# dalab/matrix-manifolds

Hardware: NVIDIA B200
Metric: spd4_pair_dist_grad_evals_per_sec (higher is better)
Workload: dtype f32

## Files before the change

matrix-manifolds_b200/csrc/gm_manifolds.cuh:

```cuda
#pragma once
#include "gm_math.cuh"

namespace gm {


template <typename T, int N, bool FAST_CHOL>
struct InvChol {
  T a[N * N];
  T l[N * N];
  T fa, fb, fc, fdet;
  GM_HD void run(const T (&x)[N * N]) {
    if constexpr (FAST_CHOL) {
      static_assert(N == 2, "closed-form Cholesky exists for 2x2 only");
      const T eps = (T)1e-8;
      T x00 = clamp_min(x[0], eps);
      fa = Num<T>::sqrt(x00);
      fb = x[1] / fa;
      fc = Num<T>::sqrt(x[3] - fb * fb + eps);
      fdet = clamp_min(fa * fc, eps);
      a[0] = fc / fdet; a[1] = (T)0; a[2] = -fb / fdet; a[3] = fa / fdet;
      l[0] = fa; l[1] = (T)0; l[2] = fb; l[3] = fc;
    } else {
      chol_lower<T, N>(x, l);
      tri_inv_lower<T, N>(l, a);
// ... 40 lines not shown
struct ClosedEig;

template <typename T>
struct ClosedEig<T, 2> {
  GM_HD static T run(const T (&m)[4], T wmin, T wmax, bool want_grad, T (&g)[4]) {
    const T eps = (T)1e-8;
    T a = m[0], b = m[3], c = m[1];
    T det = a * b - c * c;
    T h = (T)0.5 * (a + b);
    T delta = clamp_min(h * h - det, eps);
    T r = Num<T>::sqrt(delta);
    T e1 = clampv(h - r, wmin, wmax), e2 = clampv(h + r, wmin, wmax);
    T l1 = Num<T>::log(e1), l2 = Num<T>::log(e2);
    T phi = l1 * l1 + l2 * l2;
    if (want_grad) {
      T g1 = (T)2 * l1 / e1, g2 = (T)2 * l2 / e2;
      T sh = (T)0.5 * (g1 + g2);
      T dr = (g2 - g1) / (r + r);
      g[0] = sh + dr * (h - b);
      g[3] = sh + dr * (h - a);
      g[1] = g[2] = dr * c;
    }
    return phi;
  }
};

template <typename T>
struct ClosedEig<T, 3> {
  GM_HD static T run(const T (&m)[9], T wmin, T wmax, bool want_grad, T (&g)[9]) {
    const T eps = (T)1e-8;
    const T two_pi_3 = (T)2.0943951023931954923084289221863;
    T q = (m[0] + m[4] + m[8]) / (T)3;
    T y00 = m[0] - q, y11 = m[4] - q, y22 = m[8] - q;
    T y01 = m[1], y02 = m[2], y12 = m[5];
    T y10 = m[3], y20 = m[6], y21 = m[7];
    T ss = y00 * y00 + y01 * y01 + y02 * y02 + y10 * y10 + y11 * y11 + y12 * y12 + y20 * y20 + y21 * y21 +
           y22 * y22;
    T p = clamp_min(Num<T>::sqrt(ss / (T)6), eps);
    T det = y00 * y11 * y22 + (T)2 * y01 * y02 * y12 - y11 * y02 * y02 - y00 * y12 * y12 - y22 * y01 * y01;
    T den = (T)2 * p * p * p + eps;
    T r = clampv(det / den, (T)-1 + eps, (T)1 - eps);
    T phi3 = Num<T>::acos(r) / (T)3;
    T c1 = Num<T>::cos(phi3), c2 = Num<T>::cos(phi3 + two_pi_3);
    T e1 = q + (T)2 * p * c1;
    T e2 = q + (T)2 * p * c2;
    T e3 = (T)3 * q - e1 - e2;
    T f1 = clampv(e1, wmin, wmax), f2 = clampv(e2, wmin, wmax), f3 = clampv(e3, wmin, wmax);
    T l1 = Num<T>::log(f1), l2 = Num<T>::log(f2), l3 = Num<T>::log(f3);
    T phi = l1 * l1 + l2 * l2 + l3 * l3;
    if (want_grad) {
      T g1 = (T)2 * l1 / f1, g2 = (T)2 * l2 / f2, g3 = (T)2 * l3 / f3;
      T e1b = g1 - g3, e2b = g2 - g3;
      T qb = (T)3 * g3 + e1b + e2b;
      T pb = (T)2 * (e1b * c1 + e2b * c2);
      T s1 = Num<T>::sin(phi3), s2 = Num<T>::sin(phi3 + two_pi_3);
      T phib = -(T)2 * p * (e1b * s1 + e2b * s2);
      T rb = -phib / ((T)3 * Num<T>::sqrt((T)1 - r * r));
      T detb = rb / den;
      pb += -rb * (det / den) / den * (T)6 * p * p;
      T ssb = pb / ((T)2 * p) / (T)6;
      T two_ssb = ssb + ssb;
      T b00 = two_ssb * y00 + detb * (y11 * y22 - y12 * y12);
      T b11 = two_ssb * y11 + detb * (y00 * y22 - y02 * y02);
      T b22 = two_ssb * y22 + detb * (y00 * y11 - y01 * y01);
      T b01 = two_ssb * y01 + detb * ((T)2 * y02 * y12 - (T)2 * y22 * y01);
      T b02 = two_ssb * y02 + detb * ((T)2 * y01 * y12 - (T)2 * y11 * y02);
      T b12 = two_ssb * y12 + detb * ((T)2 * y01 * y02 - (T)2 * y00 * y12);
      T b10 = two_ssb * y10, b20 = two_ssb * y20, b21 = two_ssb * y21;
      T dq = (qb - (b00 + b11 + b22)) / (T)3;
      g[0] = b00 + dq; g[4] = b11 + dq; g[8] = b22 + dq;
      g[1] = g[3] = (T)0.5 * (b01 + b10);
      g[2] = g[6] = (T)0.5 * (b02 + b20);
      g[5] = g[7] = (T)0.5 * (b12 + b21);
    }
    return phi;
  }
};

template <typename T, int N, bool FAST_EIG, bool FAST_CHOL>
struct SpdAI {
  static constexpr int E = N * N;
  T wmin, wmax;

  GM_HD T dist2(const T (&x)[E], const T (&y)[E]) const {
    InvChol<T, N, FAST_CHOL> ic;
    ic.run(x);
    T m[E];
    congr_lower<T, N>(ic.a, y, m);
    T phi;
    if constexpr (FAST_EIG) {
      T dummy[E];
      phi = ClosedEig<T, N>::run(m, wmin, wmax, false, dummy);
    } else {
      T v[E], w[N];
      jacobi_eigh<T, N, false>(m, v, w);
      phi = (T)0;
      if constexpr (FAST_CHOL) {
        GM_UNROLL for (int k = 0; k < N; ++k) {
          T lg = Num<T>::log(clampv(w[k], wmin, wmax));
          phi += lg * lg;
        }
      } else {
        const T lo = Num<T>::max(wmin, Num<T>::tiny), hi = Num<T>::min(wmax, Num<T>::huge);
        GM_UNROLL for (int k = 0; k < N; ++k) {
          T lg = Num<T>::log_pos(clampv(w[k], lo, hi));
          phi += lg * lg;
        }
      }
    }
    return clamp_min(phi, wmin);
  }

  static constexpr bool kCanPrep = !FAST_EIG && !FAST_CHOL;
  static constexpr int kPrepSize = N * (N + 1) / 2;
  struct EigState {
    T wm[E];
    T cx[N], cy[N];
  };
  GM_HD void prep(const T (&x)[E], T (&ap)[kPrepSize]) const {
    InvChol<T, N, false> ic;
    ic.run(x);
    GM_UNROLL for (int i = 0; i < N; ++i)
      GM_UNROLL for (int j = 0; j <= i; ++j) ap[i * (i + 1) / 2 + j] = ic.a[i * N + j];
  }
  GM_HD T eig_forward(const T (&a)[E], const T (&y)[E], EigState& st, int max_sweeps = JacobiCfg<T>::max_sweeps,
                      bool* converged = nullptr) const {
    T m[E], w[N];
    congr_lower<T, N>(a, y, m);
    GM_UNROLL for (int i = 0; i < N; ++i)
      GM_UNROLL for (int j = 0; j < N; ++j) st.wm[i * N + j] = (j >= i) ? a[j * N + i] : (T)0;
    const bool conv = jacobi_eigh<T, N, true, false>(m, st.wm, w, max_sweeps);
    if (converged) *converged = conv;
    T phi = (T)0;
    const T lo = Num<T>::max(wmin, Num<T>::tiny), hi = Num<T>::min(wmax, Num<T>::huge);
    GM_UNROLL for (int k = 0; k < N; ++k) {
      T wc = clampv(w[k], lo, hi);
      T lg = Num<T>::log_pos(wc);
      phi += lg * lg;
      T c = Num<T>::div_fast(lg + lg, wc);
      st.cy[k] = c;
      st.cx[k] = -c * w[k];
    }
    return clamp_min(phi, wmin);
  }
  GM_HD T eig_forward_prepped(const T (&ap)[kPrepSize], const T (&y)[E], EigState& st,
                              int max_sweeps = JacobiCfg<T>::max_sweeps, bool* converged = nullptr) const {
    T a[E];
    GM_UNROLL for (int i = 0; i < N; ++i)
      GM_UNROLL for (int j = 0; j < N; ++j) a[i * N + j] = (j <= i) ? ap[i * (i + 1) / 2 + j] : (T)0;
    return eig_forward(a, y, st, max_sweeps, converged);
  }
  GM_HD void eig_backward(const EigState& st, T wgt, T (&gx)[E], T (&gy)[E]) const {
    T cx[N], cy[N];
    GM_UNROLL for (int k = 0; k < N; ++k) { cx[k] = st.cx[k] * wgt; cy[k] = st.cy[k] * wgt; }
    wdwt<T, N>(st.wm, cx, gx);
    wdwt<T, N>(st.wm, cy, gy);
  }

  GM_HD T dist2_grad(const T (&x)[E], const T (&y)[E], T (&gx)[E], T (&gy)[E]) const {
    InvChol<T, N, FAST_CHOL> ic;
    ic.run(x);
    T m[E];
    congr_lower<T, N>(ic.a, y, m);
    T phi = (T)0;
    if constexpr (!FAST_EIG && !FAST_CHOL) {
      EigState st;
      T d2 = eig_forward(ic.a, y, st);
      eig_backward(st, (T)1, gx, gy);
      return d2;
    } else {
      T g[E];
      if constexpr (FAST_EIG) {
        phi = ClosedEig<T, N>::run(m, wmin, wmax, true, g);
      } else {
        T mm[E], v[E], w[N], c[N];
        GM_UNROLL for (int k = 0; k < E; ++k) mm[k] = m[k];
        jacobi_eigh<T, N, true>(mm, v, w);
        phi = (T)0;
        GM_UNROLL for (int k = 0; k < N; ++k) {
          T wc = clampv(w[k], wmin, wmax);
          T lg = Num<T>::log(wc);
          phi += lg * lg;
          c[k] = (T)2 * lg / wc;
        }
        wdwt<T, N>(v, c, g);
      }
      congr_lowerT<T, N>(ic.a, g, gy);
      if constexpr (FAST_CHOL) {
        T ga[E], abar[E];
        matmul<T, N>(g, ic.a, ga);
        matmul<T, N>(ga, y, abar);
        GM_UNROLL for (int k = 0; k < E; ++k) abar[k] *= (T)2;
        ic.backward_closed(abar, gx);
      } else {
        T k[E], pm[E];
        matmul<T, N>(g, m, k);
        GM_UNROLL for (int i = 0; i < N; ++i)
          GM_UNROLL for (int j = 0; j <= i; ++j) {
            pm[i * N + j] = -k[i * N + j];
            pm[j * N + i] = -k[i * N + j];
          }
        congr_lowerT<T, N>(ic.a, pm, gx);
      }
    }
    return clamp_min(phi, wmin);
  }
};

template <typename T, int N, bool FAST_CHOL>
struct SpdStein {
  static constexpr int E = N * N;
  static constexpr bool kCanPrep = false;
  static constexpr int kPrepSize = 1;
  T wmin, wmax;
  struct EigState {};
  GM_HD void prep(const T (&)[E], T (&)[1]) const {}
  GM_HD T eig_forward_prepped(const T (&)[1], const T (&)[E], EigState&, int = 0, bool* = nullptr) const { return (T)0; }
  GM_HD void eig_backward(const EigState&, T, T (&)[E], T (&)[E]) const {}

  template <bool WANT_INV>
  GM_HD static T logdet_inv(const T (&x)[E], T (&inv)[E]) {
    InvChol<T, N, FAST_CHOL> ic;
    ic.run(x);
    T ld = (T)0;
    GM_UNROLL for (int k = 0; k < N; ++k) ld += Num<T>::log(Num<T>::abs(ic.l[k * N + k]));
    if (WANT_INV) {
      GM_UNROLL for (int i = 0; i < N; ++i)
        GM_UNROLL for (int j = i; j < N; ++j) {
          T s = (T)0;
          GM_UNROLL for (int k = j; k < N; ++k) s += ic.a[k * N + i] * ic.a[k * N + j];
          inv[i * N + j] = s;
          inv[j * N + i] = s;
        }
    }
    return (T)2 * ld;
  }

  GM_HD T dist2(const T (&x)[E], const T (&y)[E]) const {
    T z[E], dummy[E];
// ... 138 lines not shown
      return d * d;
    } else if constexpr (KIND == VEC_SPHERE) {
      T s = (T)0;
      for (int k = 0; k < n; ++k) s += x[k] * y[k];
      s = clampv(s, -one_m, one_m);
      T d = clamp_min(Num<T>::acos(s), eps);
      c = -(T)2 * d / Num<T>::sqrt((T)1 - s * s);
      return d * d;
    } else if constexpr (KIND == VEC_EUCLIDEAN) {
      T s = (T)0;
      for (int k = 0; k < n; ++k) { T d = y[k] - x[k]; s += d * d; }
      c = (T)2;
      return clamp_min(s, eps);
    } else {
      const T cc = *c_dev;
      c = cc;
      T x2 = (T)0, y2 = (T)0, xy = (T)0;
      for (int k = 0; k < n; ++k) { x2 += x[k] * x[k]; y2 += y[k] * y[k]; xy += x[k] * y[k]; }
      const T A = (T)1 - (T)2 * cc * xy + cc * y2;
      const T B = (T)1 - cc * x2;
      const T D = (T)1 - (T)2 * cc * xy + cc * cc * x2 * y2;
      const bool d_free = D >= (T)Kappa<T>::kMinNorm;
      const T invD = (T)1 / clamp_min(D, (T)Kappa<T>::kMinNorm);
      co.zA = -A * invD;
      co.zB = B * invD;
      T r2 = (T)0, zx = (T)0, zy = (T)0;
      for (int k = 0; k < n; ++k) {
        T z = co.zA * x[k] + co.zB * y[k];
        r2 += z * z; zx += z * x[k]; zy += z * y[k];
      }
      const T r = Num<T>::sqrt(r2);
      const T sc = Num<T>::sqrt(Num<T>::abs(cc));
      T dphi;
      const T phi = Kappa<T>::arctan_func(sc * r, cc, dphi);
      const T d = phi * (T)2 / sc;
      const T d2 = d * d;
      const T gz = (r > (T)0) ? (T)4 * d * dphi / r : (T)0;
      const T dA = -(gz * zx) * invD;
      const T dB = (gz * zy) * invD;
      const T dD = d_free ? -(gz * r2) * invD : (T)0;
      const T g_xy = -(T)2 * cc * (dA + dD);
      const T g_x2 = -cc * dB + cc * cc * y2 * dD;
      const T g_y2 = cc * dA + cc * cc * x2 * dD;
      co.p1 = co.zA * gz; co.p2 = (T)2 * g_x2; co.p3 = g_xy;
      co.q1 = co.zB * gz; co.q2 = (T)2 * g_y2;
      const T sgn = cc > (T)0 ? (T)1 : (T)-1;
      const T w = cc * r2;
      T explicit_c;
      if (sizeof(T) == 4 && Num<T>::abs(w) < (T)0.1) {
        T sres = (T)0;
        GM_UNROLL for (int k = 8; k >= 1; --k) sres = sres * w + (T)(2.0 * k / (2.0 * k + 1.0));
        explicit_c = (T)2 * d * r * r2 * sres;
      } else {
        explicit_c = ((T)4 * d * dphi * r - (T)2 * d2) / sc * (sgn * (T)0.5 / sc);
      }
      co.dc = dA * (y2 - (T)2 * xy) - dB * x2 + dD * ((T)2 * cc * x2 * y2 - (T)2 * xy) + explicit_c;
      return clamp_min(d2, eps);
    }
  }
  GM_HD void grad_elem(int k, T xk, T yk, const VecCoef<T>& co, T& gxk, T& gyk) const {
    const T c = co.c;
    if constexpr (KIND == VEC_LORENTZ) {
      T sg = (k == 0) ? c : -c;
      gxk = sg * yk; gyk = sg * xk;
    } else if constexpr (KIND == VEC_SPHERE) {
      gxk = c * yk; gyk = c * xk;
    } else if constexpr (KIND == VEC_EUCLIDEAN) {
      T d = yk - xk;
      gxk = -c * d; gyk = c * d;
    } else {
      T z = co.zA * xk + co.zB * yk;
      gxk = co.p1 * z + co.p2 * xk + co.p3 * yk;
      gyk = co.q1 * z + co.q2 * yk + co.p3 * xk;
    }
  }
};

struct LossCfg {
  int kind, inc_l1, inc_l2;
  double alpha, eps;
};

template <typename T, bool FAST = false>
GM_HD T loss_term(const LossCfg& c, T g, T m, T& dm) {
  if (c.kind == 1) {
    T d = m - g;
    dm = (T)2 * d;
    return d * d;
  }
  T t = g * (T)c.alpha;
  T v = (T)0;
  dm = (T)0;
  if (c.inc_l1) {
    T rt = FAST ? Num<T>::div_fast((T)1, t) : (T)1 / t;
    T q = FAST ? m * rt - (T)1 : m / t - (T)1;
    v += Num<T>::abs(q);
    dm += sgn0(q) * rt;
  }
  if (c.inc_l2) {
    T den = m + (T)c.eps;
    T rd = FAST ? Num<T>::div_fast((T)1, den) : (T)1 / den;
    T q = FAST ? t * rd - (T)1 : t / den - (T)1;
    v += Num<T>::abs(q);
    dm -= FAST ? sgn0(q) * t * rd * rd : sgn0(q) * t / (den * den);
  }
  return v;
}

}
```

matrix-manifolds_b200/csrc/gm_math.cuh:

```cuda
#pragma once
#include <cuda_runtime.h>
#include <math.h>
#include <float.h>

#define GM_HD __host__ __device__ __forceinline__
#ifndef GM_ROT_NEWTON
#define GM_ROT_NEWTON 1
#endif

namespace gm {

template <typename T> struct Num;
template <> struct Num<float> {
  static constexpr float eps = FLT_EPSILON;
  static constexpr float tiny = FLT_MIN;
  static constexpr float huge = FLT_MAX;
  GM_HD static float sqrt(float x) { return sqrtf(x); }
  GM_HD static float rsqrt(float x) {
#ifdef __CUDA_ARCH__
    return rsqrtf(x);
#else
    return 1.0f / sqrtf(x);
#endif
  }
  GM_HD static float rsqrt_raw(float x) {
#ifdef __CUDA_ARCH__
    float r;
    asm("rsqrt.approx.ftz.f32 %0, %1;" : "=f"(r) : "f"(x));
    return r;
#else
    return 1.0f / sqrtf(x);
#endif
  }
  GM_HD static float rcp_raw(float x) {
#ifdef __CUDA_ARCH__
    float r;
    asm("rcp.approx.ftz.f32 %0, %1;" : "=f"(r) : "f"(x));
    return r;
#else
    return 1.0f / x;
#endif
  }
  GM_HD static float div_fast(float a, float b) { return a * rcp_raw(b); }
  GM_HD static float recip(float x) {
#ifdef __CUDA_ARCH__
    float r = rcp_raw(x);
    return fmaf(r, fmaf(-x, r, 1.0f), r);
#else
    return 1.0f / x;
#endif
  }
  GM_HD static float mul_sign(float v, float d) {
#ifdef __CUDA_ARCH__
    return __uint_as_float(__float_as_uint(v) ^ (__float_as_uint(d) & 0x80000000u));
#else
    return std::signbit(d) ? -v : v;
#endif
  }
  GM_HD static void rotation(float d, float apq, float& t, float& c, float& s) {
    float two = apq + apq;
    float h2 = fmaf(two, two, fmaf(d, d, FLT_MIN));
    float h = h2 * rsqrt_raw(h2);
    float den = fabsf(d) + h;
    t = mul_sign(two, d) * rcp_raw(den);
    float x = fmaf(t, t, 1.0f);
    float r = rsqrt_raw(x);
#if GM_ROT_NEWTON
    c = r * fmaf(-0.5f * x, r * r, 1.5f);
#else
    c = r;
#endif
    s = t * c;
  }
  GM_HD static float log(float x) { return logf(x); }
  GM_HD static float log_pos(float x) {
#ifdef __CUDA_ARCH__
    int ix = __float_as_int(x);
    int e = (ix - 0x3f2aaaab) & 0xff800000;
    float m = fmaf(x, 0.0f, __int_as_float(ix - e));
    float f = m - 1.0f;
    float g = -0.12734152376651764f;
    g = fmaf(g, f, 0.13756538927555084f);
    g = fmaf(g, f, -0.12219617515802383f);
    g = fmaf(g, f, 0.1405421793460846f);
    g = fmaf(g, f, -0.16678093373775482f);
    g = fmaf(g, f, 0.2000732272863388f);
    g = fmaf(g, f, -0.24999839067459106f);
    g = fmaf(g, f, 0.33333271741867065f);
    g = fmaf(g, f, -0.5f);
    float r = fmaf(f, f * g, f);
    return fmaf((float)e, 1.1920928955078125e-07f * 0.693147180559945309f, r);
#else
    return logf(x);
#endif
  }
  GM_HD static float log1p(float x) { return log1pf(x); }
  GM_HD static float exp(float x) { return expf(x); }
  GM_HD static float acos(float x) { return acosf(x); }
  GM_HD static float atan(float x) { return atanf(x); }
  GM_HD static float tan(float x) { return tanf(x); }
  GM_HD static float tanh(float x) { return tanhf(x); }
  GM_HD static float cos(float x) { return cosf(x); }
  GM_HD static float sin(float x) { return sinf(x); }
  GM_HD static float cosh(float x) { return coshf(x); }
  GM_HD static float sinh(float x) { return sinhf(x); }
  GM_HD static float abs(float x) { return fabsf(x); }
  GM_HD static float fma(float a, float b, float c) { return fmaf(a, b, c); }
  GM_HD static float max(float a, float b) { return fmaxf(a, b); }
  GM_HD static float min(float a, float b) { return fminf(a, b); }
  GM_HD static float copysign(float a, float b) { return copysignf(a, b); }
};
template <> struct Num<double> {
  static constexpr double eps = DBL_EPSILON;
  static constexpr double tiny = DBL_MIN;
  static constexpr double huge = DBL_MAX;
  GM_HD static double sqrt(double x) { return ::sqrt(x); }
  GM_HD static double rsqrt(double x) { return 1.0 / ::sqrt(x); }
  GM_HD static double div_fast(double a, double b) { return a / b; }
  GM_HD static double recip(double x) { return 1.0 / x; }
  GM_HD static void rotation(double d, double apq, double& t, double& c, double& s) {
    double two = apq + apq;
    double den = fabs(d) + ::sqrt(d * d + two * two);
    t = (den > 0.0) ? (d >= 0.0 ? two : -two) / den : 0.0;
    c = 1.0 / ::sqrt(t * t + 1.0);
    s = t * c;
  }
  GM_HD static double log(double x) { return ::log(x); }
  GM_HD static double log_pos(double x) { return ::log(x); }
  GM_HD static double log1p(double x) { return ::log1p(x); }
  GM_HD static double exp(double x) { return ::exp(x); }
  GM_HD static double acos(double x) { return ::acos(x); }
  GM_HD static double atan(double x) { return ::atan(x); }
  GM_HD static double tan(double x) { return ::tan(x); }
  GM_HD static double tanh(double x) { return ::tanh(x); }
  GM_HD static double cos(double x) { return ::cos(x); }
  GM_HD static double sin(double x) { return ::sin(x); }
  GM_HD static double cosh(double x) { return ::cosh(x); }
  GM_HD static double sinh(double x) { return ::sinh(x); }
  GM_HD static double abs(double x) { return fabs(x); }
  GM_HD static double fma(double a, double b, double c) { return ::fma(a, b, c); }
  GM_HD static double max(double a, double b) { return fmax(a, b); }
  GM_HD static double min(double a, double b) { return fmin(a, b); }
  GM_HD static double copysign(double a, double b) { return ::copysign(a, b); }
};

template <typename T>
GM_HD T clampv(T x, T lo, T hi) {
  return x < lo ? lo : (x > hi ? hi : x);
}
template <typename T>
GM_HD T clamp_min(T x, T lo) { return x < lo ? lo : x; }
template <typename T>
GM_HD T clamp_max(T x, T hi) { return x > hi ? hi : x; }
template <typename T>
GM_HD T sgn0(T x) { return (T)((x > (T)0) - (x < (T)0)); }

#define GM_UNROLL _Pragma("unroll")

template <typename T, int N>
GM_HD void chol_lower(const T (&x)[N * N], T (&l)[N * N]) {
  GM_UNROLL for (int j = 0; j < N; ++j) {
    T s = x[j * N + j];
    GM_UNROLL for (int k = 0; k < j; ++k) s -= l[j * N + k] * l[j * N + k];
    T d = Num<T>::sqrt(s);
    l[j * N + j] = d;
    T inv = (T)1 / d;
    GM_UNROLL for (int i = j + 1; i < N; ++i) {
      T t = x[i * N + j];
      GM_UNROLL for (int k = 0; k < j; ++k) t -= l[i * N + k] * l[j * N + k];
      l[i * N + j] = t * inv;
    }
    GM_UNROLL for (int i = 0; i < j; ++i) l[i * N + j] = (T)0;
  }
}

template <typename T, int N>
GM_HD void tri_inv_lower(const T (&l)[N * N], T (&a)[N * N]) {
  GM_UNROLL for (int j = 0; j < N; ++j) {
    GM_UNROLL for (int i = 0; i < j; ++i) a[i * N + j] = (T)0;
    a[j * N + j] = (T)1 / l[j * N + j];
    GM_UNROLL for (int i = j + 1; i < N; ++i) {
      T s = (T)0;
      GM_UNROLL for (int k = j; k < i; ++k) s += l[i * N + k] * a[k * N + j];
      a[i * N + j] = -s / l[i * N + i];
    }
  }
}

template <typename T, int N>
GM_HD void congr_lower(const T (&a)[N * N], const T (&y)[N * N], T (&m)[N * N]) {
  T t[N * N];
  GM_UNROLL for (int i = 0; i < N; ++i)
    GM_UNROLL for (int j = 0; j < N; ++j) {
      T s = (T)0;
      GM_UNROLL for (int k = 0; k <= i; ++k) s += a[i * N + k] * y[k * N + j];
      t[i * N + j] = s;
    }
  GM_UNROLL for (int i = 0; i < N; ++i)
    GM_UNROLL for (int j = i; j < N; ++j) {
      T s = (T)0;
      GM_UNROLL for (int k = 0; k <= j; ++k) s += t[i * N + k] * a[j * N + k];
      m[i * N + j] = s;
      m[j * N + i] = s;
    }
}

template <typename T, int N>
GM_HD void congr_full(const T (&a)[N * N], const T (&y)[N * N], T (&m)[N * N]) {
  T t[N * N];
  GM_UNROLL for (int i = 0; i < N; ++i)
    GM_UNROLL for (int j = 0; j < N; ++j) {
      T s = (T)0;
      GM_UNROLL for (int k = 0; k < N; ++k) s += a[i * N + k] * y[k * N + j];
      t[i * N + j] = s;
    }
  GM_UNROLL for (int i = 0; i < N; ++i)
    GM_UNROLL for (int j = i; j < N; ++j) {
      T s = (T)0;
      GM_UNROLL for (int k = 0; k < N; ++k) s += t[i * N + k] * a[j * N + k];
      m[i * N + j] = s;
      m[j * N + i] = s;
    }
}

template <typename T, int N>
GM_HD void lowerT_mul(const T (&a)[N * N], const T (&v)[N * N], T (&w)[N * N]) {
  GM_UNROLL for (int i = 0; i < N; ++i)
    GM_UNROLL for (int j = 0; j < N; ++j) {
      T s = (T)0;
      GM_UNROLL for (int k = i; k < N; ++k) s += a[k * N + i] * v[k * N + j];
      w[i * N + j] = s;
    }
}

template <typename T, int N>
GM_HD void lower_mul(const T (&l)[N * N], const T (&v)[N * N], T (&w)[N * N]) {
  GM_UNROLL for (int i = 0; i < N; ++i)
    GM_UNROLL for (int j = 0; j < N; ++j) {
      T s = (T)0;
      GM_UNROLL for (int k = 0; k <= i; ++k) s += l[i * N + k] * v[k * N + j];
      w[i * N + j] = s;
    }
}

template <typename T, int N>
GM_HD void wdwt(const T (&w)[N * N], const T (&c)[N], T (&g)[N * N]) {
  GM_UNROLL for (int i = 0; i < N; ++i)
    GM_UNROLL for (int j = i; j < N; ++j) {
      T s = (T)0;
      GM_UNROLL for (int k = 0; k < N; ++k) s += (w[i * N + k] * c[k]) * w[j * N + k];
      g[i * N + j] = s;
      g[j * N + i] = s;
    }
}

template <typename T, int N>
GM_HD void matmul(const T (&a)[N * N], const T (&b)[N * N], T (&c)[N * N]) {
  GM_UNROLL for (int i = 0; i < N; ++i)
    GM_UNROLL for (int j = 0; j < N; ++j) {
      T s = (T)0;
      GM_UNROLL for (int k = 0; k < N; ++k) s += a[i * N + k] * b[k * N + j];
      c[i * N + j] = s;
    }
}

template <typename T> struct JacobiCfg;
#ifndef GM_JACOBI_F32_OFF
#define GM_JACOBI_F32_OFF 16.0f
#endif
#ifndef GM_JACOBI_F32_OFF_MAX_N
#define GM_JACOBI_F32_OFF_MAX_N 4
#endif
template <> struct JacobiCfg<float> {
  static constexpr int max_sweeps = 10;
  static constexpr float off_factor = GM_JACOBI_F32_OFF;
};
template <> struct JacobiCfg<double> {
  static constexpr int max_sweeps = 16;
  static constexpr double off_factor = 0.0625;
};

template <int N>
struct JacobiFirstCheck { static constexpr int value = N >= 4 ? 3 : (N == 3 ? 2 : 1); };

template <typename T, int N, bool WANT_V = true, bool INIT_V = true>
GM_HD bool jacobi_eigh(T (&a)[N * N], T (&v)[N * N], T (&w)[N], int max_sweeps = JacobiCfg<T>::max_sweeps) {
  if (WANT_V && INIT_V) {
    GM_UNROLL for (int i = 0; i < N; ++i)
      GM_UNROLL for (int j = 0; j < N; ++j) v[i * N + j] = (i == j) ? (T)1 : (T)0;
  }
  if (N == 1) { w[0] = a[0]; return true; }
  auto rotate = [&](const int p, const int q) {
    T apq = a[p * N + q];
    T t, c, s;
    Num<T>::rotation(a[q * N + q] - a[p * N + p], apq, t, c, s);
    if constexpr (N >= 5) {
      const T app = a[p * N + p], aqq = a[q * N + q], cs2 = (T)2 * c * s * apq;
      a[p * N + p] = c * c * app - cs2 + s * s * aqq;
      a[q * N + q] = s * s * app + cs2 + c * c * aqq;
    } else {
      a[p * N + p] = Num<T>::fma(-t, apq, a[p * N + p]);
      a[q * N + q] = Num<T>::fma(t, apq, a[q * N + q]);
    }
    a[p * N + q] = (T)0;
    a[q * N + p] = (T)0;
    GM_UNROLL for (int r = 0; r < N; ++r) {
      if (r != p && r != q) {
        T arp = a[r * N + p], arq = a[r * N + q];
        T nrp = c * arp - s * arq;
        T nrq = s * arp + c * arq;
        a[r * N + p] = nrp; a[p * N + r] = nrp;
        a[r * N + q] = nrq; a[q * N + r] = nrq;
      }
    }
    if (WANT_V) {
      GM_UNROLL for (int r = 0; r < N; ++r) {
        T vrp = v[r * N + p], vrq = v[r * N + q];
        v[r * N + p] = c * vrp - s * vrq;
        v[r * N + q] = s * vrp + c * vrq;
      }
    }
  };
  bool converged = false;
  for (int sweep = 0;; ++sweep) {
    if (sweep >= JacobiFirstCheck<N>::value || sweep >= max_sweeps) {
      T off = (T)0, dia = (T)0;
      GM_UNROLL for (int i = 0; i < N; ++i) {
        dia += a[i * N + i] * a[i * N + i];
        GM_UNROLL for (int j = i + 1; j < N; ++j) off += a[i * N + j] * a[i * N + j];
      }
      constexpr T off_factor = (N <= GM_JACOBI_F32_OFF_MAX_N) ? JacobiCfg<T>::off_factor : (T)0.0625;
      converged = off <= (Num<T>::eps * Num<T>::eps * off_factor) * dia || off < Num<T>::tiny;
      if (converged || sweep >= max_sweeps) break;
    }
    if constexpr (N == 4) {
      rotate(0, 1); rotate(2, 3);
      rotate(0, 2); rotate(1, 3);
      rotate(0, 3); rotate(1, 2);
    } else {
      GM_UNROLL for (int p = 0; p < N - 1; ++p)
        GM_UNROLL for (int q = p + 1; q < N; ++q) rotate(p, q);
    }
  }
  GM_UNROLL for (int i = 0; i < N; ++i) w[i] = a[i * N + i];
  return converged;
}

template <typename T, int R, int C>
GM_HD void jacobi_svd(T (&a)[R * C], T (&v)[C * C], T (&s)[C]) {
  GM_UNROLL for (int i = 0; i < C; ++i)
    GM_UNROLL for (int j = 0; j < C; ++j) v[i * C + j] = (i == j) ? (T)1 : (T)0;
  for (int sweep = 0; sweep < JacobiCfg<T>::max_sweeps + 4; ++sweep) {
    bool rotated = false;
    GM_UNROLL for (int p = 0; p < C - 1; ++p) {
      GM_UNROLL for (int q = p + 1; q < C; ++q) {
        T alpha = (T)0, beta = (T)0, gamma = (T)0;
        GM_UNROLL for (int r = 0; r < R; ++r) {
          alpha += a[r * C + p] * a[r * C + p];
          beta += a[r * C + q] * a[r * C + q];
          gamma += a[r * C + p] * a[r * C + q];
        }
        if (Num<T>::abs(gamma) > (Num<T>::eps * (T)0.25) * Num<T>::sqrt(alpha * beta) &&
            Num<T>::abs(gamma) > Num<T>::tiny) {
          rotated = true;
          T t, c, sn;
          Num<T>::rotation(beta - alpha, gamma, t, c, sn);
          GM_UNROLL for (int r = 0; r < R; ++r) {
            T x = a[r * C + p], y = a[r * C + q];
            a[r * C + p] = c * x - sn * y;
            a[r * C + q] = sn * x + c * y;
          }
          GM_UNROLL for (int r = 0; r < C; ++r) {
            T x = v[r * C + p], y = v[r * C + q];
            v[r * C + p] = c * x - sn * y;
            v[r * C + q] = sn * x + c * y;
          }
        }
      }
    }
    if (!rotated) break;
  }
  GM_UNROLL for (int k = 0; k < C; ++k) {
    T n2 = (T)0;
    GM_UNROLL for (int r = 0; r < R; ++r) n2 += a[r * C + k] * a[r * C + k];
    s[k] = Num<T>::sqrt(n2);
  }
}

template <typename T>
__device__ __forceinline__ T warp_sum(T v) {
  GM_UNROLL for (int o = 16; o > 0; o >>= 1) v += __shfl_xor_sync(0xffffffffu, v, o);
  return v;
}

__device__ __forceinline__ void block_accumulate(double v, double* dst, double* red) {
  v = warp_sum(v);
  int lane = threadIdx.x & 31, wid = threadIdx.x >> 5;
  if (lane == 0) red[wid] = v;
  __syncthreads();
  if (wid == 0) {
    int nw = (blockDim.x + 31) >> 5;
    double s = lane < nw ? red[lane] : 0.0;
    s = warp_sum(s);
    if (lane == 0 && dst != nullptr) atomicAdd(dst, s);
  }
  __syncthreads();
}

}
```

matrix-manifolds_b200/csrc/gm_pairs_spd.cu:

```cuda
#include "gm_product.cuh"

#ifndef GM_N
#error "compile with -DGM_N=<matrix size>"
#endif

namespace gm {

template <class Op, typename T, int KMODE>
__global__ void __launch_bounds__(128)
spd_pair_kernel(Op op, PairSpec ps, const T* __restrict__ xa, const T* __restrict__ xb,
                const T* __restrict__ gout, T coef, T* __restrict__ ga, T* __restrict__ gb,
                T* __restrict__ out_d2, TargetSpec tg, LossCfg lc, T scale_sp, double* __restrict__ acc) {
  constexpr int E = Op::E;
  __shared__ double red[2][4];
  long long k = (long long)blockIdx.x * blockDim.x + threadIdx.x;
  bool active = k < ps.P;
  long long ra = -1, rb = -1;
  double loss_v = 0.0, gd2_v = 0.0;
  T gx[E], gy[E];
  if (active) {
    decode_pair(ps, k, ra, rb);
    T x[E], y[E];
    load_row<T, E>(xa, ra, x);
    load_row<T, E>(xb, rb, y);
    if constexpr (KMODE == K_FWD) {
      out_d2[k] = op.dist2(x, y);
    } else {
      T d2 = op.dist2_grad(x, y, gx, gy);
      T w;
      if constexpr (KMODE == K_BWD) {
        w = coef * gout[k];
      } else {
        T g = fetch_target_ps<T>(ps, tg, k, ra, rb);
        T m = scale_sp * d2;
        T dm;
        T lv = loss_term<T>(lc, g, m, dm);
        loss_v = (double)lv;
        gd2_v = (double)dm * (double)d2;
        w = dm * scale_sp;
        if (out_d2) out_d2[k] = d2;
      }
      GM_UNROLL for (int e = 0; e < E; ++e) { gx[e] *= w; gy[e] *= w; }
    }
  }
  if constexpr (KMODE != K_FWD) {
    if (ps.mode == GM_PAIRS_ELEMENTWISE) {
      if (active) {
        store_row<T, E>(ga, ra, gx);
        store_row<T, E>(gb, rb, gy);
      }
    } else {
      warp_accumulate_row<T, E>(ga, ra, gx);
      warp_accumulate_row<T, E>(gb, rb, gy);
    }
  }
  if constexpr (KMODE == K_FUSED) {
    block_accumulate(loss_v, acc, red[0]);
    block_accumulate(gd2_v, acc + 1, red[1]);
  }
}

template <int BYTES>
__device__ __forceinline__ void cp_async(void* smem, const void* gmem) {
  unsigned s = (unsigned)__cvta_generic_to_shared(smem);
  if constexpr (BYTES == 16)
    asm volatile("cp.async.cg.shared.global [%0], [%1], 16;\n" ::"r"(s), "l"(gmem) : "memory");
  else if constexpr (BYTES == 8)
    asm volatile("cp.async.ca.shared.global [%0], [%1], 8;\n" ::"r"(s), "l"(gmem) : "memory");
  else
    asm volatile("cp.async.ca.shared.global [%0], [%1], 4;\n" ::"r"(s), "l"(gmem) : "memory");
}
__device__ __forceinline__ void cp_async_commit() { asm volatile("cp.async.commit_group;\n" ::: "memory"); }
__device__ __forceinline__ void cp_async_wait_all() { asm volatile("cp.async.wait_group 0;\n" ::: "memory"); }
template <int PENDING>
__device__ __forceinline__ void cp_async_wait_group() { asm volatile("cp.async.wait_group %0;\n" ::"n"(PENDING) : "memory"); }

template <typename T, int E, int STAGES = 2>
struct RowStage {
  static constexpr int ROWB = E * (int)sizeof(T);
  static constexpr int CPB = (ROWB % 16 == 0) ? 16 : ((ROWB % 8 == 0) ? 8 : 4);
  static constexpr int NCH = ROWB / CPB;
  static constexpr int THREADS = 128;
  static constexpr int BYTES = STAGES * 2  * ROWB * THREADS;
  __device__ __forceinline__ static char* slot(char* base, int s, int r, int c, int t) {
    return base + ((((s * 2 + r) * NCH + c) * THREADS + t) * CPB);
  }
  __device__ __forceinline__ static void issue(char* base, int s, int r, int t, const T* row) {
    const char* g = reinterpret_cast<const char*>(row);
    GM_UNROLL for (int c = 0; c < NCH; ++c) cp_async<CPB>(slot(base, s, r, c, t), g + c * CPB);
  }
  __device__ __forceinline__ static void read(char* base, int s, int r, int t, T (&out)[E]) {
    GM_UNROLL for (int c = 0; c < NCH; ++c) {
      if constexpr (CPB == 16) {
        float4 v = *reinterpret_cast<const float4*>(slot(base, s, r, c, t));
        const T* tv = reinterpret_cast<const T*>(&v);
        GM_UNROLL for (int j = 0; j < 16 / (int)sizeof(T); ++j) out[c * (16 / (int)sizeof(T)) + j] = tv[j];
      } else if constexpr (CPB == 8) {
        float2 v = *reinterpret_cast<const float2*>(slot(base, s, r, c, t));
        const T* tv = reinterpret_cast<const T*>(&v);
        GM_UNROLL for (int j = 0; j < 8 / (int)sizeof(T); ++j) out[c * (8 / (int)sizeof(T)) + j] = tv[j];
      } else {
        out[c] = *reinterpret_cast<const T*>(slot(base, s, r, c, t));
      }
    }
  }
};

struct PairCursor {
  long long a, pos;
  int slot;
  __device__ __forceinline__ void init(const PairSpec& ps, long long k0) {
    if (ps.mode == GM_PAIRS_TRIU && k0 < ps.P) {
      long long b;
      triu_decode(k0 + ps.k0, ps.B, a, b);
      pos = b - a - 1;
    } else {
      a = -1; pos = 0; slot = 0;
    }
  }
// ... 171 lines not shown
    v[D] = locate(32 * D, kq);
    if (v[D]) load_rows(kq, ra[D], rb[D], hopn);
  }
  [[maybe_unused]] int hs = SPEC ? (32 * (D + 1)) / (int)chunk : 0;
  [[maybe_unused]] int ho = SPEC ? 32 * (D + 1) - hs * (int)chunk : 0;

  double loss_v = 0.0, gd2_v = 0.0;
  row_t acc_row = kNoRow;
  T gacc[EU];
  GM_UNROLL for (int e = 0; e < EU; ++e) gacc[e] = (T)0;
  row_t prep_row = kNoRow;
  T ap[Op::kPrepSize];

  auto flush = [&]() {
    if (acc_row != kNoRow) {
      GM_UNROLL for (int e = 0; e < EU; ++e) gacc[e] = warp_sum(gacc[e]);
      if (lane == 0) {
        T gfull[E];
        GM_UNROLL for (int i = 0; i < N; ++i)
          GM_UNROLL for (int j = i; j < N; ++j) {
            gfull[i * N + j] = gacc[i * N - i * (i - 1) / 2 + (j - i)];
            gfull[j * N + i] = gfull[i * N + j];
          }
        long long lr;
        T* gbase = grow(ga, acc_row, lr);
        atomic_add_row<T, E>(gbase, lr, gfull);
      }
      GM_UNROLL for (int e = 0; e < EU; ++e) gacc[e] = (T)0;
      acc_row = kNoRow;
    }
  };

  const int t_end = (nseg > 1 && wbase - lane < ps.seg_len) ? nseg * (int)chunk : 0;
  while (nseg > 1 ? tc < t_end : __any_sync(full, v[0])) {
    cp_async_wait_group<D - 1>();
    const bool v0 = v[0];
    const row_t ra0 = ra[0], rb0 = rb[0];
    const raw_t tg0 = tgq[0];
    T x[E], y[E];
    if (v0) {
      Stage::read(stage_mem, stage, 1, tid, y);
      if (!Op::kCanPrep || ra0 != prep_row) Stage::read(stage_mem, stage, 0, tid, x);
    }
    tgq[D] = 0;
    if (v[D]) {
      long long kq = 0;
      if (KMODE == K_BWD || !hopsP) locate(tc + 32 * D, kq);
      tgq[D] = (sampled && hopsP) ? (raw_t)hopn : fetch_scalar(kq, ra[D], rb[D]);
      if (rawj) rb[D] &= (row_t)0x00ffffffu;
      int sn = stage + D;
      if (sn > D) sn -= D + 1;
      Stage::issue(stage_mem, sn, 0, tid, xrow(xa, ra[D]));
      Stage::issue(stage_mem, sn, 1, tid, xrow(xb, rb[D]));
    }
    cp_async_commit();
    ahead.advance(ps);
    long long kh = 0;
    if constexpr (SPEC != 0) {
      v[D + 1] = locate_so(hs, ho, kh);
      ho += 32;
      if (ho >= (int)chunk) { ho -= (int)chunk; ++hs; }
    } else {
      v[D + 1] = locate(tc + 32 * (D + 1), kh);
    }
    ra[D + 1] = kNoRow; rb[D + 1] = kNoRow;
    unsigned hop_next = 0;
    if (v[D + 1]) load_rows(kh, ra[D + 1], rb[D + 1], hop_next);

    T gx[E], gy[E];
    if (v0) {
      T d2, w;
      [[maybe_unused]] typename Op::EigState st;
      if constexpr (Op::kCanPrep) {
        if (ra0 != prep_row) { op.prep(x, ap); prep_row = ra0; }
        d2 = op.eig_forward_prepped(ap, y, st);
      } else {
        d2 = op.dist2_grad(x, y, gx, gy);
      }
      if constexpr (KMODE == K_BWD) {
        w = coef * scalar_value(tg0);
      } else {
        T m = scale_sp * d2;
        T dm;
        T lv = loss_term<T, true>(lc, scalar_value(tg0), m, dm);
        loss_v += (double)lv;
        gd2_v += (double)dm * (double)d2;
        w = dm * scale_sp;
        if (out_d2) {
          long long k0 = 0;
          locate(tc, k0);
          out_d2[k0] = d2;
        }
      }
      if constexpr (Op::kCanPrep) {
        op.eig_backward(st, w, gx, gy);
      } else {
        GM_UNROLL for (int e = 0; e < E; ++e) { gx[e] *= w; gy[e] *= w; }
      }
      long long lrb;
      T* gbb = grow(gb, rb0, lrb);
      atomic_add_row<T, E>(gbb, lrb, gy);
    }
    {
      row_t r0 = __shfl_sync(full, ra0, 0);
      bool uniform = __all_sync(full, v0 && ra0 == r0);
      if (uniform && r0 == acc_row) {
        GM_UNROLL for (int i = 0; i < N; ++i)
          GM_UNROLL for (int j = i; j < N; ++j) gacc[i * N - i * (i - 1) / 2 + (j - i)] += gx[i * N + j];
      } else {
        flush();
        if (uniform) {
          acc_row = r0;
          GM_UNROLL for (int i = 0; i < N; ++i)
            GM_UNROLL for (int j = i; j < N; ++j) gacc[i * N - i * (i - 1) / 2 + (j - i)] = gx[i * N + j];
        } else if (v0) {
          long long lra;
          T* gba = grow(ga, ra0, lra);
          atomic_add_row<T, E>(gba, lra, gx);
        }
      }
    }
    tc += 32;
    GM_UNROLL for (int q = 0; q < D + 1; ++q) { ra[q] = ra[q + 1]; rb[q] = rb[q + 1]; v[q] = v[q + 1]; }
    GM_UNROLL for (int q = 0; q < D; ++q) tgq[q] = tgq[q + 1];
    hopn = hop_next;
    stage = (stage == D) ? 0 : stage + 1;
  }
  flush();
  if constexpr (KMODE == K_FUSED) {
    block_accumulate(loss_v, acc, red[0]);
    block_accumulate(gd2_v, acc + 1, red[1]);
  }
}

template <class Op, typename T>
static int launch_op(const Op& op, const PairArgs& a) {
  if (a.ps.P <= 0) return 0;
  if (a.px) return a.sh.log2w >= 0 ? GM_EUNSUPPORTED : launch_product<SpdLead<Op>, T>(SpdLead<Op>{op}, a);
  const int threads = 128;
  long long blocks = (a.ps.P + threads - 1) / threads;
  if (blocks > 0x7fffffffLL) return GM_EINVAL;
  dim3 grid((unsigned)blocks), block(threads);
  const T* xa = (const T*)a.xa;
  const T* xb = (const T*)a.xb;
#ifndef GM_MINB_F32
#define GM_MINB_F32 4
#endif
#ifndef GM_PF_DEPTH
#define GM_PF_DEPTH 1
#endif
  constexpr int MINB = sizeof(T) == 4 ? GM_MINB_F32 : 2;
  constexpr int DEPTH = (RowStage<T, Op::E, GM_PF_DEPTH + 1>::BYTES + 3 * 1024) * MINB <= 224 * 1024 ? GM_PF_DEPTH : 1;
  using Stage = RowStage<T, Op::E, DEPTH + 1>;
  if (a.kmode != K_FWD && a.ps.mode != GM_PAIRS_ELEMENTWISE && RowStage<T, Op::E, 2>::BYTES <= 64 * 1024) {
    int dev = 0, sms = 0, occ = 0;
    cudaGetDevice(&dev);
    cudaDeviceGetAttribute(&sms, cudaDevAttrMultiProcessorCount, dev);
    auto launch_stream = [&](auto kern, auto spec_kern, const T* gout, T coef, T* out_d2, T scale, double* acc) -> int {
      cudaFuncSetAttribute(kern, cudaFuncAttributeMaxDynamicSharedMemorySize, Stage::BYTES);
      cudaOccupancyMaxActiveBlocksPerMultiprocessor(&occ, kern, threads, Stage::BYTES);
      if (occ < 1) occ = 1;
      long long max_blocks = (long long)sms * occ;
      long long want = (a.ps.P + threads - 1) / threads;
      long long nb = want < max_blocks ? want : max_blocks;
      long long warps = nb * (threads / 32);
      PairSpec ps = a.ps;
      if (ps.mode != GM_PAIRS_LIST || ps.nseg < 2 || ps.P < ps.nseg * 32LL * warps) ps.nseg = 1;
// ... 83 lines not shown
```

Before: 15.25 billion.

## Use packed f32x2 FMA for 4x4 SPD congruence, eigvec rotations and backward

Adds an f32x2 type backed by Blackwell packed fma/mul/add.rn.f32x2 PTX. The 4x4 float SPD path uses it for a specialized congruence, Jacobi eigenvector rotations stored as row pairs, a two-lane polynomial log, and the W diag W^T gradient reconstruction, so two scalar FP32 operations issue as one instruction. It also changes the loss sign test to compensate for rounding error in m, and adds a diagnostic script. The risks are packing overhead through 64-bit moves, higher register pressure, and slightly different rounding from the custom log.

```diff
diff --git a/_diag.py b/_diag.py
--- /dev/null
+++ b/_diag.py
@@ -0,0 +1,45 @@
+import os, sys, torch
+sys.path[:0] = ['tests', 'oracle', 'matrix-manifolds_b200']
+import helpers_hotpath as H
+from graphembed import _ops, _lib as L
+from graphembed.manifolds import SymmetricPositiveDefinite
+DEV = torch.device('cuda', 0); MAX_SQ = 64.0
+S = float(torch.nn.functional.softplus(torch.tensor(0.5)))
+x, cls, _ = H.point_table(4, {H.CA: 2048, H.CB: 2048}, seed=21)
+gen = torch.Generator().manual_seed(22)
+B = 1536
+nodes = torch.randperm(x.shape[0], generator=gen)[:B]
+ia, ib = torch.triu_indices(B, B, 1)
+k0 = int(torch.nonzero(ia == 100)[0]) + 37
+P = ia.numel() - k0 - 1234
+I, J = nodes[ia[k0:k0 + P]], nodes[ib[k0:k0 + P]]
+h = torch.randint(1, 9, (x.shape[0], x.shape[0]), generator=gen, dtype=torch.uint8)
+h = torch.triu(h, 1) + torch.triu(h, 1).T
+ref = H.PairReference(x, I, J, 4)
+pcls = H.pair_classes(cls, I, J); rcls = H.row_classes(cls, (I, J), pcls)
+dense = (h.float() ** 2) / MAX_SQ
+xd = x.to(DEV)
+pairs = _ops.PairSet.triu(B, nodes=nodes.to(torch.int32).to(DEV), device=DEV, k0=k0, P=P)
+grad = torch.zeros_like(xd)
+acc, d2 = _ops.pairs_loss_fused(SymmetricPositiveDefinite(4).spec, xd, pairs, _ops.TargetSpec.dense(dense.to(DEV)),
+                                _ops.LossSpec(L.GM_LOSS_QUOTIENT, True, True, 1.0, 0.5), S, grad, want_d2=True)
+d2 = d2.cpu(); grad = grad.cpu()
+g = dense[I, J].double()
+w = H.loss_weights('quotient', g, d2, S)[2]
+chk = H.Checker(torch.float32, os.environ['TAG'])
+chk.grad([(grad, [(I, 'gx'), (J, 'gy')])], ref, w, [rcls])
+print(chk.report())
+g64 = torch.zeros(x.shape, dtype=torch.float64); A = torch.zeros(x.shape[0], dtype=torch.float64)
+for rows, side in ((I, 'gx'), (J, 'gy')):
+    c = w.view(-1, 1, 1) * getattr(ref, side + '_64'); g64.index_add_(0, rows, c); A.index_add_(0, rows, H._item_max(c))
+loc = H._item_max(grad.double() - g64) / A.clamp(min=1e-300)
+top = torch.topk(loc, 4)
+m64 = S * d2.double()
+q1 = m64 / g - 1.0; q2 = g / (m64 + 0.5) - 1.0
+near = (q1.abs() < 3e-6) | (q2.abs() < 3e-6)
+print('pairs within 3e-6 of a kink:', int(near.sum()))
+for r, v in zip(top.indices.tolist(), top.values.tolist()):
+    sel = near & ((I == r) | (J == r))
+    ks = torch.nonzero(sel).flatten().tolist()
+    info = [(k, f'q1={q1[k]:.2e}', f'q2={q2[k]:.2e}', f'|w contrib|/A={(w[k].abs() * H._item_max(ref.gx_64[k:k+1] if I[k]==r else ref.gy_64[k:k+1])[0] / A[r]).item():.2e}') for k in ks]
+    print(f'row {r} cls {int(rcls[r])} loc err {v:.2e} near-kink pairs {info}')
diff --git a/matrix-manifolds_b200/csrc/gm_manifolds.cuh b/matrix-manifolds_b200/csrc/gm_manifolds.cuh
--- a/matrix-manifolds_b200/csrc/gm_manifolds.cuh
+++ b/matrix-manifolds_b200/csrc/gm_manifolds.cuh
@@ -146,10 +146,20 @@
   static constexpr int E = N * N;
   T wmin, wmax;
 
+  static constexpr bool kPacked = sizeof(T) == 4 && N == 4 && !FAST_EIG && !FAST_CHOL;
+
   GM_HD T dist2(const T (&x)[E], const T (&y)[E]) const {
     InvChol<T, N, FAST_CHOL> ic;
     ic.run(x);
     T m[E];
+    if constexpr (kPacked) {
+      T ap[kPrepSize], v[E], w[N];
+      pack_factor(ic.a, ap);
+      congr4(ap, y, m);
+      jacobi_eigh<T, N, false>(m, v, w);
+      f32x2 wc[2], lg[2];
+      return clamp_min(log_pairs(w, wc, lg), wmin);
+    }
     congr_lower<T, N>(ic.a, y, m);
     T phi;
     if constexpr (FAST_EIG) {
@@ -177,18 +187,90 @@
 
   static constexpr bool kCanPrep = !FAST_EIG && !FAST_CHOL;
   static constexpr int kPrepSize = N * (N + 1) / 2;
-  struct EigState {
+  struct EigStateScalar {
     T wm[E];
     T cx[N], cy[N];
   };
+  struct EigStatePacked {
+    f32x2 wp[8];
+    f32x2 cx[2], cy[2];
+  };
+  using EigState = typename std::conditional<kPacked, EigStatePacked, EigStateScalar>::type;
+
+  GM_HD static void pack_factor(const T (&a)[E], T (&ap)[kPrepSize]) {
+    if constexpr (kPacked) {
+      const int src[kPrepSize] = {0, 4, 8, 12, 9, 13, 10, 14, 5, 15};
+      GM_UNROLL for (int e = 0; e < kPrepSize; ++e) ap[e] = a[src[e]];
+    } else {
+      GM_UNROLL for (int i = 0; i < N; ++i)
+        GM_UNROLL for (int j = 0; j <= i; ++j) ap[i * (i + 1) / 2 + j] = a[i * N + j];
+    }
+  }
+  GM_HD static void congr4(const float (&ap)[10], const float (&y)[16], float (&m)[16]) {
+    const f32x2 a0{ap[0], ap[1]}, b0{ap[2], ap[3]}, b1{ap[4], ap[5]}, b2{ap[6], ap[7]};
+    const float a11 = ap[8], a33 = ap[9];
+    f32x2 t0[4], t1[4];
+    GM_UNROLL for (int j = 0; j < 4; ++j) {
+      t0[j] = mul2(a0, y[j]);
+      t0[j].y = fmaf(a11, y[4 + j], t0[j].y);
+      t1[j] = fma2(b2, y[8 + j], fma2(b1, y[4 + j], mul2(b0, y[j])));
+      t1[j].y = fmaf(a33, y[12 + j], t1[j].y);
+    }
+    const f32x2 m00 = mul2(t0[0], ap[0]);
+    const f32x2 m01 = fma2(t0[1], a11, mul2(t0[0], ap[1]));
+    const f32x2 m02 = fma2(t0[2], ap[6], fma2(t0[1], ap[4], mul2(t0[0], ap[2])));
+    const f32x2 m03 = fma2(t0[3], a33, fma2(t0[2], ap[7], fma2(t0[1], ap[5], mul2(t0[0], ap[3]))));
+    const f32x2 m22 = fma2(t1[2], ap[6], fma2(t1[1], ap[4], mul2(t1[0], ap[2])));
+    const f32x2 m23 = fma2(t1[3], a33, fma2(t1[2], ap[7], fma2(t1[1], ap[5], mul2(t1[0], ap[3]))));
+    m[0] = m00.x; m[1] = m01.x; m[2] = m02.x; m[3] = m03.x;
+    m[5] = m01.y; m[6] = m02.y; m[7] = m03.y;
+    m[10] = m22.x; m[11] = m23.x;
+    m[15] = m23.y;
+    GM_UNROLL for (int i = 1; i < 4; ++i)
+      GM_UNROLL for (int j = 0; j < i; ++j) m[i * 4 + j] = m[j * 4 + i];
+  }
+  GM_HD T log_pairs(const float (&w)[4], f32x2 (&wc)[2], f32x2 (&lg)[2]) const {
+    const T lo = Num<T>::max(wmin, Num<T>::tiny), hi = Num<T>::min(wmax, Num<T>::huge);
+    GM_UNROLL for (int h = 0; h < 2; ++h) {
+      wc[h] = f32x2{clampv(w[2 * h], lo, hi), clampv(w[2 * h + 1], lo, hi)};
+      lg[h] = log_pos2(wc[h]);
+    }
+    const f32x2 p = fma2(lg[1], lg[1], mul2(lg[0], lg[0]));
+    return p.x + p.y;
+  }
+  GM_HD static void wdwt4(const f32x2 (&wp)[8], const f32x2 (&c)[2], float (&g)[16]) {
+    f32x2 u[8];
+    GM_UNROLL for (int h = 0; h < 2; ++h)
+      GM_UNROLL for (int k = 0; k < 4; ++k) u[4 * h + k] = mul2(wp[4 * h + k], (k & 1) ? c[k >> 1].y : c[k >> 1].x);
+    GM_UNROLL for (int i = 0; i < 4; ++i)
+      GM_UNROLL for (int h = i >> 1; h < 2; ++h) {
+        auto U = [&](int k) { return (i & 1) ? u[4 * (i >> 1) + k].y : u[4 * (i >> 1) + k].x; };
+        f32x2 r = mul2(wp[4 * h], U(0));
+        GM_UNROLL for (int k = 1; k < 4; ++k) r = fma2(wp[4 * h + k], U(k), r);
+        g[i * 4 + 2 * h] = r.x;
+        g[i * 4 + 2 * h + 1] = r.y;
+      }
+    GM_UNROLL for (int i = 1; i < 4; ++i)
+      GM_UNROLL for (int j = 0; j < i; ++j) g[i * 4 + j] = g[j * 4 + i];
+  }
+
   GM_HD void prep(const T (&x)[E], T (&ap)[kPrepSize]) const {
     InvChol<T, N, false> ic;
     ic.run(x);
-    GM_UNROLL for (int i = 0; i < N; ++i)
-      GM_UNROLL for (int j = 0; j <= i; ++j) ap[i * (i + 1) / 2 + j] = ic.a[i * N + j];
+    pack_factor(ic.a, ap);
   }
   GM_HD T eig_forward(const T (&a)[E], const T (&y)[E], EigState& st, int max_sweeps = JacobiCfg<T>::max_sweeps,
                       bool* converged = nullptr) const {
+    if constexpr (kPacked) {
+      T ap[kPrepSize];
+      pack_factor(a, ap);
+      return eig_forward_prepped(ap, y, st, max_sweeps, converged);
+    } else {
+      return eig_forward_scalar(a, y, st, max_sweeps, converged);
+    }
+  }
+  GM_HD T eig_forward_scalar(const T (&a)[E], const T (&y)[E], EigStateScalar& st, int max_sweeps,
+                             bool* converged) const {
     T m[E], w[N];
     congr_lower<T, N>(a, y, m);
     GM_UNROLL for (int i = 0; i < N; ++i)
@@ -209,16 +291,42 @@
   }
   GM_HD T eig_forward_prepped(const T (&ap)[kPrepSize], const T (&y)[E], EigState& st,
                               int max_sweeps = JacobiCfg<T>::max_sweeps, bool* converged = nullptr) const {
-    T a[E];
-    GM_UNROLL for (int i = 0; i < N; ++i)
-      GM_UNROLL for (int j = 0; j < N; ++j) a[i * N + j] = (j <= i) ? ap[i * (i + 1) / 2 + j] : (T)0;
-    return eig_forward(a, y, st, max_sweeps, converged);
+    if constexpr (kPacked) {
+      T m[E], w[N];
+      congr4(ap, y, m);
+      st.wp[0] = f32x2{ap[0], 0.0f};  st.wp[1] = f32x2{ap[1], ap[8]};
+      st.wp[2] = f32x2{ap[2], ap[4]}; st.wp[3] = f32x2{ap[3], ap[5]};
+      st.wp[4] = f32x2{0.0f, 0.0f};   st.wp[5] = f32x2{0.0f, 0.0f};
+      st.wp[6] = f32x2{ap[6], 0.0f};  st.wp[7] = f32x2{ap[7], ap[9]};
+      const bool conv = jacobi_eigh4_rowpairs(m, st.wp, w, max_sweeps);
+      if (converged) *converged = conv;
+      f32x2 wc[2], lg[2];
+      const T phi = log_pairs(w, wc, lg);
+      GM_UNROLL for (int h = 0; h < 2; ++h) {
+        const f32x2 c = mul2(add2(lg[h], lg[h]), f32x2{Num<T>::rcp_raw(wc[h].x), Num<T>::rcp_raw(wc[h].y)});
+        st.cy[h] = c;
+        st.cx[h] = mul2(c, f32x2{w[2 * h], w[2 * h + 1]});
+      }
+      return clamp_min(phi, wmin);
+    } else {
+      T a[E];
+      GM_UNROLL for (int i = 0; i < N; ++i)
+        GM_UNROLL for (int j = 0; j < N; ++j) a[i * N + j] = (j <= i) ? ap[i * (i + 1) / 2 + j] : (T)0;
+      return eig_forward_scalar(a, y, st, max_sweeps, converged);
+    }
   }
   GM_HD void eig_backward(const EigState& st, T wgt, T (&gx)[E], T (&gy)[E]) const {
-    T cx[N], cy[N];
-    GM_UNROLL for (int k = 0; k < N; ++k) { cx[k] = st.cx[k] * wgt; cy[k] = st.cy[k] * wgt; }
-    wdwt<T, N>(st.wm, cx, gx);
-    wdwt<T, N>(st.wm, cy, gy);
+    if constexpr (kPacked) {
+      const f32x2 cx[2] = {mul2(st.cx[0], -wgt), mul2(st.cx[1], -wgt)};
+      const f32x2 cy[2] = {mul2(st.cy[0], wgt), mul2(st.cy[1], wgt)};
+      wdwt4(st.wp, cx, gx);
+      wdwt4(st.wp, cy, gy);
+    } else {
+      T cx[N], cy[N];
+      GM_UNROLL for (int k = 0; k < N; ++k) { cx[k] = st.cx[k] * wgt; cy[k] = st.cy[k] * wgt; }
+      wdwt<T, N>(st.wm, cx, gx);
+      wdwt<T, N>(st.wm, cy, gy);
+    }
   }
 
   GM_HD T dist2_grad(const T (&x)[E], const T (&y)[E], T (&gx)[E], T (&gy)[E]) const {
@@ -523,7 +631,7 @@
 };
 
 template <typename T, bool FAST = false>
-GM_HD T loss_term(const LossCfg& c, T g, T m, T& dm) {
+GM_HD T loss_term(const LossCfg& c, T g, T m, T& dm, T m_err = (T)0) {
   if (c.kind == 1) {
     T d = m - g;
     dm = (T)2 * d;
@@ -536,7 +644,7 @@
     T rt = FAST ? Num<T>::div_fast((T)1, t) : (T)1 / t;
     T q = FAST ? m * rt - (T)1 : m / t - (T)1;
     v += Num<T>::abs(q);
-    dm += sgn0(q) * rt;
+    dm += sgn0((m - t) + m_err) * rt;
   }
   if (c.inc_l2) {
     T den = m + (T)c.eps;
diff --git a/matrix-manifolds_b200/csrc/gm_math.cuh b/matrix-manifolds_b200/csrc/gm_math.cuh
--- a/matrix-manifolds_b200/csrc/gm_math.cuh
+++ b/matrix-manifolds_b200/csrc/gm_math.cuh
@@ -2,6 +2,7 @@
 #include <cuda_runtime.h>
 #include <math.h>
 #include <float.h>
+#include <type_traits>
 
 #define GM_HD __host__ __device__ __forceinline__
 #ifndef GM_ROT_NEWTON
@@ -144,6 +145,75 @@
   GM_HD static double copysign(double a, double b) { return ::copysign(a, b); }
 };
 
+struct __align__(8) f32x2 {
+  float x, y;
+};
+GM_HD f32x2 make_f32x2(float x, float y) { return f32x2{x, y}; }
+#ifdef __CUDA_ARCH__
+__device__ __forceinline__ unsigned long long pk2(f32x2 a) {
+  unsigned long long r;
+  asm("mov.b64 %0, {%1, %2};" : "=l"(r) : "f"(a.x), "f"(a.y));
+  return r;
+}
+__device__ __forceinline__ f32x2 upk2(unsigned long long r) {
+  f32x2 a;
+  asm("mov.b64 {%0, %1}, %2;" : "=f"(a.x), "=f"(a.y) : "l"(r));
+  return a;
+}
+#endif
+GM_HD f32x2 fma2(f32x2 a, f32x2 b, f32x2 c) {
+#ifdef __CUDA_ARCH__
+  unsigned long long d;
+  asm("fma.rn.f32x2 %0, %1, %2, %3;" : "=l"(d) : "l"(pk2(a)), "l"(pk2(b)), "l"(pk2(c)));
+  return upk2(d);
+#else
+  return f32x2{fmaf(a.x, b.x, c.x), fmaf(a.y, b.y, c.y)};
+#endif
+}
+GM_HD f32x2 mul2(f32x2 a, f32x2 b) {
+#ifdef __CUDA_ARCH__
+  unsigned long long d;
+  asm("mul.rn.f32x2 %0, %1, %2;" : "=l"(d) : "l"(pk2(a)), "l"(pk2(b)));
+  return upk2(d);
+#else
+  return f32x2{a.x * b.x, a.y * b.y};
+#endif
+}
+GM_HD f32x2 add2(f32x2 a, f32x2 b) {
+#ifdef __CUDA_ARCH__
+  unsigned long long d;
+  asm("add.rn.f32x2 %0, %1, %2;" : "=l"(d) : "l"(pk2(a)), "l"(pk2(b)));
+  return upk2(d);
+#else
+  return f32x2{a.x + b.x, a.y + b.y};
+#endif
+}
+GM_HD f32x2 fma2(f32x2 a, float s, f32x2 c) { return fma2(a, f32x2{s, s}, c); }
+GM_HD f32x2 fma2(f32x2 a, float s, float c) { return fma2(a, f32x2{s, s}, f32x2{c, c}); }
+GM_HD f32x2 mul2(f32x2 a, float s) { return mul2(a, f32x2{s, s}); }
+GM_HD f32x2 add2(f32x2 a, float s) { return add2(a, f32x2{s, s}); }
+
+GM_HD f32x2 log_pos2(f32x2 x) {
+#ifdef __CUDA_ARCH__
+  const int ix0 = __float_as_int(x.x), ix1 = __float_as_int(x.y);
+  const int e0 = (ix0 - 0x3f2aaaab) & 0xff800000, e1 = (ix1 - 0x3f2aaaab) & 0xff800000;
+  f32x2 m = fma2(x, 0.0f, f32x2{__int_as_float(ix0 - e0), __int_as_float(ix1 - e1)});
+  f32x2 f = add2(m, -1.0f);
+  f32x2 g = fma2(f, -0.12734152376651764f, 0.13756538927555084f);
+  g = fma2(g, f, f32x2{-0.12219617515802383f, -0.12219617515802383f});
+  g = fma2(g, f, f32x2{0.1405421793460846f, 0.1405421793460846f});
+  g = fma2(g, f, f32x2{-0.16678093373775482f, -0.16678093373775482f});
+  g = fma2(g, f, f32x2{0.2000732272863388f, 0.2000732272863388f});
+  g = fma2(g, f, f32x2{-0.24999839067459106f, -0.24999839067459106f});
+  g = fma2(g, f, f32x2{0.33333271741867065f, 0.33333271741867065f});
+  g = fma2(g, f, f32x2{-0.5f, -0.5f});
+  f32x2 r = fma2(f, mul2(f, g), f);
+  return fma2(f32x2{(float)e0, (float)e1}, 1.1920928955078125e-07f * 0.693147180559945309f, r);
+#else
+  return f32x2{Num<float>::log_pos(x.x), Num<float>::log_pos(x.y)};
+#endif
+}
+
 template <typename T>
 GM_HD T clampv(T x, T lo, T hi) {
   return x < lo ? lo : (x > hi ? hi : x);
@@ -283,12 +353,8 @@
 template <int N>
 struct JacobiFirstCheck { static constexpr int value = N >= 4 ? 3 : (N == 3 ? 2 : 1); };
 
-template <typename T, int N, bool WANT_V = true, bool INIT_V = true>
-GM_HD bool jacobi_eigh(T (&a)[N * N], T (&v)[N * N], T (&w)[N], int max_sweeps = JacobiCfg<T>::max_sweeps) {
-  if (WANT_V && INIT_V) {
-    GM_UNROLL for (int i = 0; i < N; ++i)
-      GM_UNROLL for (int j = 0; j < N; ++j) v[i * N + j] = (i == j) ? (T)1 : (T)0;
-  }
+template <typename T, int N, class VRot>
+GM_HD bool jacobi_sweeps(T (&a)[N * N], T (&w)[N], int max_sweeps, VRot&& vrot) {
   if (N == 1) { w[0] = a[0]; return true; }
   auto rotate = [&](const int p, const int q) {
     T apq = a[p * N + q];
@@ -313,13 +379,7 @@
         a[r * N + q] = nrq; a[q * N + r] = nrq;
       }
     }
-    if (WANT_V) {
-      GM_UNROLL for (int r = 0; r < N; ++r) {
-        T vrp = v[r * N + p], vrq = v[r * N + q];
-        v[r * N + p] = c * vrp - s * vrq;
-        v[r * N + q] = s * vrp + c * vrq;
-      }
-    }
+    vrot(p, q, c, s);
   };
   bool converged = false;
   for (int sweep = 0;; ++sweep) {
@@ -344,6 +404,34 @@
   }
   GM_UNROLL for (int i = 0; i < N; ++i) w[i] = a[i * N + i];
   return converged;
+}
+
+template <typename T, int N, bool WANT_V = true, bool INIT_V = true>
+GM_HD bool jacobi_eigh(T (&a)[N * N], T (&v)[N * N], T (&w)[N], int max_sweeps = JacobiCfg<T>::max_sweeps) {
+  if (WANT_V && INIT_V) {
+    GM_UNROLL for (int i = 0; i < N; ++i)
+      GM_UNROLL for (int j = 0; j < N; ++j) v[i * N + j] = (i == j) ? (T)1 : (T)0;
+  }
+  return jacobi_sweeps<T, N>(a, w, max_sweeps, [&](const int p, const int q, const T c, const T s) {
+    if (WANT_V) {
+      GM_UNROLL for (int r = 0; r < N; ++r) {
+        T vrp = v[r * N + p], vrq = v[r * N + q];
+        v[r * N + p] = c * vrp - s * vrq;
+        v[r * N + q] = s * vrp + c * vrq;
+      }
+    }
+  });
+}
+
+GM_HD bool jacobi_eigh4_rowpairs(float (&a)[16], f32x2 (&b)[8], float (&w)[4],
+                                 int max_sweeps = JacobiCfg<float>::max_sweeps) {
+  return jacobi_sweeps<float, 4>(a, w, max_sweeps, [&](const int p, const int q, const float c, const float s) {
+    GM_UNROLL for (int h = 0; h < 2; ++h) {
+      const f32x2 bp = b[4 * h + p], bq = b[4 * h + q];
+      b[4 * h + p] = fma2(bp, c, mul2(bq, -s));
+      b[4 * h + q] = fma2(bp, s, mul2(bq, c));
+    }
+  });
 }
 
 template <typename T, int R, int C>
diff --git a/matrix-manifolds_b200/csrc/gm_pairs_spd.cu b/matrix-manifolds_b200/csrc/gm_pairs_spd.cu
--- a/matrix-manifolds_b200/csrc/gm_pairs_spd.cu
+++ b/matrix-manifolds_b200/csrc/gm_pairs_spd.cu
@@ -34,7 +34,7 @@
         T g = fetch_target_ps<T>(ps, tg, k, ra, rb);
         T m = scale_sp * d2;
         T dm;
-        T lv = loss_term<T>(lc, g, m, dm);
+        T lv = loss_term<T>(lc, g, m, dm, Num<T>::fma(scale_sp, d2, -m));
         loss_v = (double)lv;
         gd2_v = (double)dm * (double)d2;
         w = dm * scale_sp;
@@ -372,7 +372,7 @@
       } else {
         T m = scale_sp * d2;
         T dm;
-        T lv = loss_term<T, true>(lc, scalar_value(tg0), m, dm);
+        T lv = loss_term<T, true>(lc, scalar_value(tg0), m, dm, Num<T>::fma(scale_sp, d2, -m));
         loss_v += (double)lv;
         gd2_v += (double)dm * (double)d2;
         w = dm * scale_sp;
```

Result: faster. 15.55 billion, median of 6 (+2.0%).
